# alexj94/future_urban_scene_generation

Measured on AMD Instinct MI355X. Metric: synthesised vehicle crops/sec @256x256, higher is better.
Workload: dtype f32 tensors; conv contraction as 3 fp16 MFMA products of scaled (hi, lo) operand splits, f32 accumulate (error vs fp64 <= 1.3x the exact-f32 MFMA kernel's: observed 0.96-1.27x over 12 operand scales x 5 layers; range-guarded; exact-f32 leg in precision_legs)

## Files before the change

### future_urban_scene_generation_amd/_lib.py

```python
from __future__ import annotations

import ctypes as C
import os

_HERE = os.path.dirname(os.path.abspath(__file__))
LIB_PATH = os.environ.get("FUSG_LIB", os.path.join(_HERE, "libfusg.so"))


class FusgUnavailable(RuntimeError):
    pass


class FusgError(RuntimeError):
    pass


class Tensor(C.Structure):
    _fields_ = [("data", C.c_void_p),
                ("n", C.c_int64), ("c", C.c_int64), ("h", C.c_int64), ("w", C.c_int64),
                ("sn", C.c_int64), ("sc", C.c_int64), ("sh", C.c_int64), ("sw", C.c_int64),
                ("dtype", C.c_int32), ("_pad", C.c_int32)]


class ConvDesc(C.Structure):
# ... 5 lines not shown
                ("stride", C.c_int32), ("upsample", C.c_int32), ("pad_mode", C.c_int32), ("pre_op", C.c_int32),
                ("act", C.c_int32), ("store_mode", C.c_int32), ("qh", C.c_int32), ("qw", C.c_int32),
                ("nphase", C.c_int32), ("out_sy", C.c_int32), ("out_sx", C.c_int32),
                ("out_oy", C.c_int32 * 4), ("out_ox", C.c_int32 * 4),
                ("dst_c_off", C.c_int32), ("tile", C.c_int32), ("ksplit", C.c_int32), ("precision", C.c_int32),
                ("wpack_h", C.c_void_p),
                ("kh", C.c_int32), ("kw", C.c_int32), ("dil", C.c_int32), ("pad_h", C.c_int32), ("pad_w", C.c_int32),
                ("wfrag_order", C.c_int32), ("wfrag", C.c_void_p), ("stats_out", C.c_void_p),
                ("tile_list", C.c_void_p), ("tile_count", C.c_int32), ("q_oy", C.c_int32), ("q_ox", C.c_int32),
                ("stats_slots", C.c_int32),
                ("wscale", C.c_void_p), ("status", C.c_void_p), ("wfrag_bf16", C.c_void_p), ("wfrag_f32", C.c_void_p),
                ("splitk_counters", C.c_void_p), ("splitk_counters_len", C.c_int32), ("tap_sparse", C.c_int32)]


class BneckDesc(C.Structure):
    _fields_ = [("x", Tensor), ("res", Tensor), ("dst", Tensor),
                ("pre_scale", C.c_void_p), ("pre_shift", C.c_void_p),
                ("w1frag", C.c_void_p), ("bias1", C.c_void_p), ("wscale1", C.c_void_p),
                ("w2frag", C.c_void_p), ("bias2", C.c_void_p), ("wscale2", C.c_void_p),
                ("w3frag", C.c_void_p), ("bias3", C.c_void_p), ("wscale3", C.c_void_p),
                ("status", C.c_void_p), ("planes", C.c_int32), ("exact_f32", C.c_int32)]


class RespairDesc(C.Structure):
    _fields_ = [("x", Tensor), ("s1", Tensor), ("kb", Tensor), ("kc", Tensor),
                ("w_in", C.c_void_p), ("bias_in", C.c_void_p),
                ("wfragA", C.c_void_p), ("biasA", C.c_void_p), ("wscaleA", C.c_void_p),
                ("wfragB", C.c_void_p), ("biasB", C.c_void_p), ("wscaleB", C.c_void_p),
                ("wfrag_b", C.c_void_p), ("bias_b", C.c_void_p), ("wscale_b", C.c_void_p),
                ("wfrag_c", C.c_void_p), ("bias_c", C.c_void_p), ("wscale_c", C.c_void_p),
                ("status", C.c_void_p), ("channels", C.c_int32), ("entry", C.c_int32),
                ("cin", C.c_int32), ("kpad_in", C.c_int32), ("tap_order", C.c_int32), ("_pad", C.c_int32)]


class HgHeadDesc(C.Structure):
    _fields_ = [("y_in", Tensor), ("x", Tensor), ("score", Tensor), ("dst", Tensor),
                ("wfrag_fc", C.c_void_p), ("bias_fc", C.c_void_p), ("wscale_fc", C.c_void_p),
                ("wfrag_score", C.c_void_p), ("bias_score", C.c_void_p), ("wscale_score", C.c_void_p),
                ("wfrag_join", C.c_void_p), ("bias_join", C.c_void_p), ("wscale_join", C.c_void_p),
                ("status", C.c_void_p), ("join", C.c_int32), ("_pad", C.c_int32)]


class PackSpec(C.Structure):
    _fields_ = [(n, C.c_int32) for n in ("cout", "cin", "kh", "kw", "c0", "stride", "pad", "dil", "upsample", "cin_pad")]


# ... 1 lines not shown
    _fields_ = [("cout_pad", C.c_int32), ("k_pad", C.c_int32), ("c0k", C.c_int32), ("c1k", C.c_int32),
                ("wfrag_order", C.c_int32), ("_pad", C.c_int32), ("wpack_floats", C.c_int64), ("ktab_ints", C.c_int64),
                ("wpack_h_halves", C.c_int64), ("wfrag_halves", C.c_int64)]


F32, U8, I32 = 0, 1, 2
PAD_ZERO, PAD_REFLECT, PAD_REPLICATE = 0, 1, 2
PRE_NONE, PRE_RELU, PRE_ELU, PRE_AFFINE_RELU, PRE_AFFINE = 0, 1, 2, 3, 4
ACT_NONE, ACT_RELU, ACT_TANH, ACT_SIGMOID, ACT_TANH01 = 0, 1, 2, 3, 4
STORE_NORMAL, STORE_D2S, STORE_S2D = 0, 1, 2
PREC_F32, PREC_F16X3, PREC_EMU_BF16, PREC_EMU_BF16X2, PREC_BF16 = 0, 1, 2, 3, 4
MAX_FRAMES = 64
TILE_AUTO, TILE_128x128, TILE_128x64, TILE_128x32, TILE_64x64, TILE_64x128 = 0, 1, 2, 3, 4, 5

_TP = C.POINTER(Tensor)
_SIGS = {
    "fusg_conv2d": (C.c_int, [C.POINTER(ConvDesc), C.c_void_p]),
    "fusg_conv2d_plan": (C.c_int64, [C.POINTER(ConvDesc)]),
    "fusg_conv2d_route": (C.c_int, [C.POINTER(ConvDesc)]),
    "fusg_set_route_batch": (C.c_int, [C.c_int32]),
    "fusg_route_batch": (C.c_int32, []),
    "fusg_conv2d_route_order": (C.c_int, [C.POINTER(ConvDesc), C.POINTER(C.c_int32 * 4)]),
    "fusg_hg_bottleneck": (C.c_int, [C.POINTER(BneckDesc), C.c_void_p]),
    "fusg_vunet_respair": (C.c_int, [C.POINTER(RespairDesc), C.c_void_p]),
    "fusg_hg_head": (C.c_int, [C.POINTER(HgHeadDesc), C.c_void_p]),
    "fusg_conv2d_entry_nin": (C.c_int, [C.POINTER(ConvDesc), C.POINTER(ConvDesc), C.c_void_p]),
    "fusg_conv2d_entry_nin_route": (C.c_int, [C.POINTER(ConvDesc), C.POINTER(ConvDesc)]),
    "fusg_chan_stats": (C.c_int, [_TP, C.c_void_p, C.c_int32, C.c_void_p]),
    "fusg_in_finalize": (C.c_int, [_TP, C.c_void_p, C.c_int32, C.c_float, C.c_void_p, C.c_void_p, C.c_void_p]),
    "fusg_ln_finalize": (C.c_int, [_TP, C.c_void_p, C.c_int32, C.c_float, C.c_void_p, C.c_void_p, C.c_void_p,
                                   C.c_void_p, C.c_void_p]),
    "fusg_in_finalize_slots": (C.c_int, [C.c_void_p, C.c_int32, C.c_int32, C.c_int32, C.c_float, C.c_void_p, C.c_void_p, C.c_void_p]),
    "fusg_ln_finalize_slots": (C.c_int, [C.c_void_p, C.c_int32, C.c_int32, C.c_int32, C.c_float, C.c_void_p, C.c_void_p,
                                         C.c_void_p, C.c_void_p, C.c_void_p]),
    "fusg_affine_act": (C.c_int, [_TP, C.c_void_p, C.c_void_p, C.c_int64, C.c_int32, _TP, _TP, C.c_void_p]),
    "fusg_maxpool2": (C.c_int, [_TP, _TP, C.c_void_p]),
    "fusg_upsample2_add": (C.c_int, [_TP, _TP, _TP, C.c_void_p]),
    "fusg_copy4d": (C.c_int, [_TP, _TP, C.c_int32, C.c_void_p]),
    "fusg_add4d": (C.c_int, [_TP, _TP, _TP, C.c_void_p]),
    "fusg_space_to_depth2": (C.c_int, [_TP, _TP, C.c_void_p]),
    "fusg_depth_to_space2": (C.c_int, [_TP, _TP, C.c_void_p]),
    "fusg_ec_inputs": (C.c_int, [_TP, _TP, _TP, _TP, C.c_int32, C.c_void_p]),
    "fusg_hshift_sum": (C.c_int, [_TP, C.c_void_p, C.c_int32, C.c_int32, C.c_int32, C.c_int32, _TP, C.c_void_p]),
    "fusg_argmax_hw": (C.c_int, [_TP, C.c_void_p, C.c_void_p]),
    "fusg_to_image_u8": (C.c_int, [_TP, _TP, C.c_void_p]),
    "fusg_merge_u8": (C.c_int, [_TP, _TP, _TP, _TP, C.c_void_p]),
# ... 43 lines not shown
    "fusg_plan_destroy": (None, [C.c_void_p]),
    "fusg_plan_begin": (C.c_int, [C.c_void_p]),
    "fusg_plan_end": (C.c_int, [C.c_void_p]),
    "fusg_plan_add_dependency": (C.c_int, [C.c_void_p, C.c_void_p, C.c_void_p]),
    "fusg_plan_add_h2d": (C.c_int, [C.c_void_p, C.c_void_p, C.c_void_p, C.c_int64, C.c_int32, C.c_int64, C.c_void_p]),
    "fusg_plan_next_slot": (C.c_int, [C.c_void_p]),
    "fusg_plan_size": (C.c_int64, [C.c_void_p]),
    "fusg_plan_run": (C.c_int, [C.c_void_p]),
    "fusg_plan_streams": (C.c_int32, [C.c_void_p]),
    "fusg_plan_run_mt": (C.c_int, [C.c_void_p]),
    "fusg_plan_graph_capture": (C.c_int, [C.c_void_p, C.c_void_p, C.c_int32]),
    "fusg_plan_graph_nodes": (C.c_int64, [C.c_void_p]),
    "fusg_plan_graph_slot": (C.c_int, [C.c_void_p]),
    "fusg_plan_graph_launch": (C.c_int, [C.c_void_p, C.c_void_p]),
    "fusg_pack_conv_sizes": (C.c_int, [C.POINTER(PackSpec), C.POINTER(PackSizes)]),
    "fusg_pack_conv_weights": (C.c_int, [C.POINTER(PackSpec)] + [C.c_void_p] * 8),
    "fusg_version": (C.c_int, []),
    "fusg_last_error": (C.c_char_p, []),
    "fusg_last_conv_kernel": (C.c_int, []),
    "fusg_arch": (C.c_char_p, []),
    "fusg_sizeof_tensor": (C.c_int, []),
    "fusg_sizeof_conv_desc": (C.c_int, []),
    "fusg_sizeof_bneck_desc": (C.c_int, []),
    "fusg_sizeof_respair_desc": (C.c_int, []),
    "fusg_sizeof_hg_head_desc": (C.c_int, []),
    "fusg_prof_enable": (None, [C.c_int]),
    "fusg_prof_reset": (None, []),
    "fusg_prof_read": (C.c_int, [C.c_int, C.POINTER(C.c_double), C.POINTER(C.c_int64), C.POINTER(C.c_double)]),
}
EXPORTS = tuple(_SIGS.keys())

ROUTE_BATCH_ENV = int(os.environ.get("FUSG_ROUTE_BATCH", "0") or 0)

_lib = None


def lib():
    global _lib
    if _lib is None:
        if not os.path.exists(LIB_PATH):
            raise FusgUnavailable(
                f"{LIB_PATH} not found: build it with `python -c 'import __graft_entry__ as g; g.build()'` "
                "(hipcc --offload-arch=gfx950).  There is no CPU fallback.")
        import torch
        try:
            h = C.CDLL(LIB_PATH)
        except OSError as e:
            raise FusgUnavailable(f"cannot load {LIB_PATH}: {e}") from e
        for name, (res, args) in _SIGS.items():
            fn = getattr(h, name)
            fn.restype = res
            fn.argtypes = args
        if (h.fusg_sizeof_tensor() != C.sizeof(Tensor) or h.fusg_sizeof_conv_desc() != C.sizeof(ConvDesc)
                or h.fusg_sizeof_bneck_desc() != C.sizeof(BneckDesc)
                or h.fusg_sizeof_respair_desc() != C.sizeof(RespairDesc)
                or h.fusg_sizeof_hg_head_desc() != C.sizeof(HgHeadDesc)):
            raise FusgUnavailable("libfusg.so struct layout differs from the ctypes mirror (stale build?)")
        if ROUTE_BATCH_ENV and h.fusg_set_route_batch(ROUTE_BATCH_ENV) < 0:
            raise FusgError(f"FUSG_ROUTE_BATCH={ROUTE_BATCH_ENV}: {h.fusg_last_error().decode()}")
        _lib = h
    return _lib


def check(rc: int, what: str = "") -> None:
    if rc != 0:
        msg = lib().fusg_last_error()
        raise FusgError(f"{what}: rc={rc}: {msg.decode() if msg else ''}")
```

### future_urban_scene_generation_amd/csrc/common.h

```cpp
#pragma once
#include <hip/hip_runtime.h>
#include <functional>
#include <memory>
#include <tuple>
#include <utility>
#include <stdint.h>
#include <stdio.h>
#include <string.h>
#include "../../include/fusg.h"

namespace fusg {

void set_error(const char* fmt, ...);
void note_conv_kernel(int kind);

#define FUSG_CHECK(cond, ...)                         \
    do {                                              \
        if (!(cond)) {                                \
            fusg::set_error(__VA_ARGS__);             \
            return FUSG_ERR_INVALID;                  \
        }                                             \
    } while (0)

#define FUSG_LAUNCH_CHECK(what)                                                    \
// ... 42 lines not shown

template <class A> struct SavedArg {
    A a;
    explicit SavedArg(A v) : a(v) {}
    A get() const { return a; }
};
template <> struct SavedArg<const fusg_tensor*> {
    bool has; fusg_tensor t;
    explicit SavedArg(const fusg_tensor* p) : has(p != nullptr), t(p ? *p : fusg_tensor{}) {}
    const fusg_tensor* get() const { return has ? &t : nullptr; }
};
template <> struct SavedArg<const fusg_conv_desc*> {
    bool has; fusg_conv_desc d;
    explicit SavedArg(const fusg_conv_desc* p) : has(p != nullptr), d(p ? *p : fusg_conv_desc{}) {}
    const fusg_conv_desc* get() const { return has ? &d : nullptr; }
};

template <> struct SavedArg<const fusg_bneck_desc*> {
    bool has; fusg_bneck_desc d;
    explicit SavedArg(const fusg_bneck_desc* p) : has(p != nullptr), d(p ? *p : fusg_bneck_desc{}) {}
    const fusg_bneck_desc* get() const { return has ? &d : nullptr; }
};

template <> struct SavedArg<const fusg_respair_desc*> {
    bool has; fusg_respair_desc d;
    explicit SavedArg(const fusg_respair_desc* p) : has(p != nullptr), d(p ? *p : fusg_respair_desc{}) {}
    const fusg_respair_desc* get() const { return has ? &d : nullptr; }
};

template <> struct SavedArg<const fusg_hg_head_desc*> {
    bool has; fusg_hg_head_desc d;
    explicit SavedArg(const fusg_hg_head_desc* p) : has(p != nullptr), d(p ? *p : fusg_hg_head_desc{}) {}
    const fusg_hg_head_desc* get() const { return has ? &d : nullptr; }
};

template <class... A>
int plan_dispatch(int (*impl)(A..., void*), void* stream, A... a) {
    if (plan_recording()) {
        auto saved = std::make_shared<std::tuple<SavedArg<A>...>>(SavedArg<A>(a)...);
        const int32_t rb = route_batch_now();
        plan_append((hipStream_t)stream, [impl, saved, rb](hipStream_t s) {
            RouteBatchScope scope(rb);
            return std::apply([&](const SavedArg<A>&... sv) { return impl(sv.get()..., (void*)s); }, *saved);
        });
    }
    return impl(a..., stream);
// ... 9 lines not shown
```

### future_urban_scene_generation_amd/csrc/conv_bneck.hip

```cpp
#include "conv_kernel_h3.h"

namespace fusg {

struct BneckK {
    const float* x; const float* res; float* dst;
    long xsn, xsh, xsw, rsn, rsh, rsw, dsn, dsh, dsw;
    const float* pre_scale; const float* pre_shift;
    const _Float16* w1; const _Float16* w2; const _Float16* w3;
    const float* b1; const float* b2; const float* b3;
    const float* s1; const float* s2; const float* s3;
    const float* zeros;
    int* status;
    int B, H, W, Cin, tiles_x, tiles_y;
    int touch_w;
};

constexpr int BN_HP = 100;
constexpr int BN_SROWS = 112;
constexpr size_t bneck_lds(int planes) { return (size_t)(2 * BN_SROWS * 32 + 2 * (planes / 32) * BN_HP * 32) * sizeof(_Float16); }

template <int CT> struct WFrag { h8 f[CT][2]; };

#ifdef FUSG_BNECK_STAMPS
__device__ unsigned long long g_bneck_stamps[64 * 12];
#define FUSG_STAMP(i) do { if (threadIdx.x == 0 && blockIdx.x < 64) g_bneck_stamps[blockIdx.x * 12 + (i)] = __builtin_amdgcn_s_memtime(); } while (0)
#define FUSG_STAMP_RT(i) do { if (threadIdx.x == 0 && blockIdx.x < 64) g_bneck_stamps[blockIdx.x * 12 + (i)] = __builtin_amdgcn_s_memrealtime(); } while (0)
#else
#define FUSG_STAMP(i) do {} while (0)
#define FUSG_STAMP_RT(i) do {} while (0)
#endif

__device__ __forceinline__ f32x4 mfma16(const h8 a, const h8 b, const f32x4 c) {
    return __builtin_amdgcn_mfma_f32_16x16x32_f16(a, b, c, 0, 0, 0);
}

template <int P>
__global__ __launch_bounds__(256, 2) void hg_bneck_h3(const BneckK k) {
    constexpr int NCH = P / 32;
    constexpr int CT1 = P / 64, CT3 = P / 32;
    extern __shared__ __attribute__((aligned(16))) _Float16 smem_h[];
    _Float16* Sh = smem_h;
    _Float16* Sl = Sh + BN_SROWS * 32;
    _Float16* Th = Sl + BN_SROWS * 32;
    _Float16* Tl = Th + NCH * BN_HP * 32;
    _Float16* Uh = Th;
    _Float16* Ul = Th + NCH * 64 * 32;

    const int t = threadIdx.x, lane = t & 63, wave = t >> 6;
    const int lp = lane & 15, lg = lane >> 4;
    FUSG_STAMP_RT(8);
    FUSG_STAMP(0);
    const int tile = xcd_tile();
    const int tpi = k.tiles_x * k.tiles_y;
    const int b = tile / tpi, t2 = tile - b * tpi;
    const int ty = t2 / k.tiles_x, tx = t2 - ty * k.tiles_x;
    const int oy0 = ty * 8, ox0 = tx * 8;
    float amax = 0.f;
    const float ninf = -__builtin_inff();

// ... 214 lines not shown
        for (int i = 0; i < 4; ++i) { xh[i] = *(const h8*)(Uh + c * 2048 + i * 512 + sfrag); xl[i] = *(const h8*)(Ul + c * 2048 + i * 512 + sfrag); }
        h8 bs[CT3];
#pragma unroll
        for (int j = 0; j < CT3; ++j) bs[j] = scale_m11(F.f[j][0]);
#pragma unroll
        for (int term = 0; term < 3; ++term)
#pragma unroll
            for (int i = 0; i < 4; ++i)
#pragma unroll
                for (int j = 0; j < CT3; ++j)
                    acc3[i][j] = mfma16(term == 0 ? F.f[j][0] : term == 1 ? F.f[j][1] : bs[j], term == 2 ? xl[i] : xh[i], acc3[i][j]);
    };
#pragma unroll
    for (int c = 0; c < NCH; c += 2) {
        load_w(v1, k.w3, c + 1, 2 * NCH, wave * CT3);
        compute3(v0, c);
        if (c + 2 < NCH) load_w(v0, k.w3, c + 2, 2 * NCH, wave * CT3);
        compute3(v1, c + 1);
    }

    FUSG_STAMP(6);
    if (amax >= F16X3_LIMIT && k.status) *k.status = 1;

#pragma unroll
    for (int i = 0; i < 4; ++i) {
        const int oy = oy0 + 2 * i + prow, ox = ox0 + pcol;
        if (oy >= k.H || ox >= k.W) continue;
        const float* rp = k.res + (long)b * k.rsn + (long)oy * k.rsh + (long)ox * k.rsw;
        float* dp = k.dst + (long)b * k.dsn + (long)oy * k.dsh + (long)ox * k.dsw;
#pragma unroll
        for (int j = 0; j < CT3; ++j) {
            const int n0 = (wave * CT3 + j) * 16 + lg * 4;
            const f32x4 bias = *(const f32x4*)(k.b3 + n0), wsc = *(const f32x4*)(k.s3 + n0);
            const f32x4 r = *(const f32x4*)(rp + n0);
            f32x4 v;
#pragma unroll
            for (int e = 0; e < 4; ++e) v[e] = fmaf(acc3[i][j][e], wsc[e], bias[e]) + r[e];
            *(f32x4*)(dp + n0) = v;
        }
    }
    FUSG_STAMP(7);
    FUSG_STAMP_RT(9);
}


template <int CT> struct WFragF { f32x4 f[CT][2]; };
// ... 205 lines not shown
#pragma unroll
    for (int i = 0; i < 4; ++i) {
        const int oy = oy0 + 2 * i + prow, ox = ox0 + pcol;
        if (oy >= k.H || ox >= k.W) continue;
        const float* rp = k.res + (long)b * k.rsn + (long)oy * k.rsh + (long)ox * k.rsw;
        float* dp = k.dst + (long)b * k.dsn + (long)oy * k.dsh + (long)ox * k.dsw;
#pragma unroll
        for (int j = 0; j < CT3; ++j) {
            const int n0 = (wave * CT3 + j) * 16 + lg * 4;
            const f32x4 bias = *(const f32x4*)(k.b3 + n0);
            const f32x4 r = *(const f32x4*)(rp + n0);
            f32x4 v;
#pragma unroll
            for (int e = 0; e < 4; ++e) v[e] = (acc3[i][j][e] + bias[e]) + r[e];
            *(f32x4*)(dp + n0) = v;
        }
    }
}

}

using namespace fusg;

static int bneck_impl(const fusg_bneck_desc* d, void* stream) {
    hipStream_t s = (hipStream_t)stream;
    FUSG_CHECK(d != nullptr, "hg_bottleneck: null descriptor");
    const fusg_tensor& x = d->x;
    const int P = d->planes;
    FUSG_CHECK(P == 128 || P == 64, "hg_bottleneck: planes %d (64 and 128 are built)", d->planes);
    FUSG_CHECK(is_nhwc(x) && x.c % 32 == 0 && x.c >= 32 && x.c <= 4096, "hg_bottleneck: x must be NHWC-physical f32 with c %% 32 == 0");
    FUSG_CHECK(is_nhwc(d->res) && is_nhwc(d->dst) && same_nhw(x, d->res) && same_nhw(x, d->dst) && d->res.c == 2 * P &&
               d->dst.c == 2 * P, "hg_bottleneck: res / dst must be NHWC-physical f32 [n, 2 * planes, h, w] like x");
    FUSG_CHECK(x.data != d->dst.data && d->res.data != d->dst.data, "hg_bottleneck: dst must not alias x or res (neighbouring patches read x's halo)");
    const bool f32 = d->exact_f32 == 1;
    FUSG_CHECK(d->exact_f32 == 0 || d->exact_f32 == 1, "hg_bottleneck: exact_f32 %d", d->exact_f32);
    const void* ptrs[] = {d->pre_scale, d->pre_shift, d->w1frag, d->bias1, d->w2frag, d->bias2, d->w3frag, d->bias3};
    for (const void* p : ptrs) FUSG_CHECK(p && (((uintptr_t)p) & 15) == 0, "hg_bottleneck: a parameter array is missing or not 16-byte aligned");
    if (!f32) {
        const void* sp[] = {d->wscale1, d->wscale2, d->wscale3};
        for (const void* p : sp) FUSG_CHECK(p && (((uintptr_t)p) & 15) == 0, "hg_bottleneck: a weight-scale array is missing or not 16-byte aligned");
        FUSG_CHECK(d->status != nullptr, "hg_bottleneck: status word missing");
    }
    FUSG_CHECK(x.n * x.h * x.w * x.sw < (1L << 40) && x.n >= 1 && x.h >= 1 && x.w >= 1, "hg_bottleneck: extent");
    BneckK k;
    memset(&k, 0, sizeof(k));
    k.x = (const float*)x.data; k.res = (const float*)d->res.data; k.dst = (float*)d->dst.data;
    k.xsn = x.sn; k.xsh = x.sh; k.xsw = x.sw;
    k.rsn = d->res.sn; k.rsh = d->res.sh; k.rsw = d->res.sw;
    k.dsn = d->dst.sn; k.dsh = d->dst.sh; k.dsw = d->dst.sw;
    k.pre_scale = d->pre_scale; k.pre_shift = d->pre_shift;
    k.w1 = (const _Float16*)d->w1frag; k.w2 = (const _Float16*)d->w2frag; k.w3 = (const _Float16*)d->w3frag;
    k.b1 = d->bias1; k.b2 = d->bias2; k.b3 = d->bias3;
    k.s1 = d->wscale1; k.s2 = d->wscale2; k.s3 = d->wscale3;
    k.status = d->status;
    k.zeros = zero_line();
    if (!k.zeros) { set_error("hg_bottleneck: cannot allocate the zero line"); return FUSG_ERR_LAUNCH; }
    k.B = (int)x.n; k.H = (int)x.h; k.W = (int)x.w; k.Cin = (int)x.c;
    k.tiles_x = (k.W + 7) / 8; k.tiles_y = (k.H + 7) / 8;
    const long wgs = (long)k.B * k.tiles_x * k.tiles_y;
    FUSG_CHECK(wgs < (1L << 31), "hg_bottleneck: grid");
    const void* fn = f32 ? (P == 128 ? (const void*)hg_bneck_f32<128> : (const void*)hg_bneck_f32<64>)
                         : (P == 128 ? (const void*)hg_bneck_h3<128> : (const void*)hg_bneck_h3<64>);
    const size_t lds = bneck_lds(P) + TOUCH_LDS_BYTES;
    k.touch_w = env_switches().no_touch ? 0 : 1;
    const double M = (double)x.n * x.h * x.w;
    prof_begin(0, s, 2.0 * M * ((double)x.c * P + 9.0 * P * P + 2.0 * P * P));
    const hipError_t e = launch_kernel(fn, dim3((unsigned)wgs), lds, (int)lds, k, s);
    prof_end(0, s);
    if (e != hipSuccess) { set_error("hg_bottleneck launch: %s", hipGetErrorString(e)); return FUSG_ERR_LAUNCH; }
    note_conv_kernel(FUSG_CONV_BNECK);
    return FUSG_OK;
}
extern "C" int fusg_hg_bottleneck(const fusg_bneck_desc* d, void* stream) { return fusg::plan_dispatch(bneck_impl, stream, d); }
#ifdef FUSG_BNECK_STAMPS
extern "C" int fusg_debug_bneck_stamps(unsigned long long* out) {
    return hipMemcpyFromSymbol(out, HIP_SYMBOL(fusg::g_bneck_stamps), sizeof(unsigned long long) * 64 * 12) == hipSuccess ? 0 : 1;
}
#endif
```

### future_urban_scene_generation_amd/ops.py

```python
from __future__ import annotations

import ctypes as C
from typing import Optional, Tuple

import torch

from . import _lib as L
from .pack import ConvPlan

_DT = {torch.float32: L.F32, torch.uint8: L.U8, torch.int32: L.I32}

import os as _os
import numpy as _np


def _env_set(name: str) -> bool:
    return name in _os.environ


_PREC = {"f32": L.PREC_F32, "f16x3": L.PREC_F16X3,
         "bf16": L.PREC_BF16,
         "emu_bf16": L.PREC_EMU_BF16, "emu_bf16x2": L.PREC_EMU_BF16X2}
_EMU_BITS = {"emu_bf16": 8, "emu_bf16x2": 16}

# ... 445 lines not shown
        d.stats_slots = int(buf.shape[1])
    L.check(lib.fusg_conv2d(C.byref(d), stream_ptr()), "conv2d")
    return (out, stats) if want_stats else out


def bottleneck_ok(p: dict, x: torch.Tensor, precision: Optional[str] = None) -> bool:
    prec = precision or PRECISION
    if prec not in ("f16x3", "f32") or _env_set("FUSG_NO_BNECK") or (prec == "f32" and (_env_set("FUSG_NO_BNECK_F32") or _env_set("FUSG_NO_F32_HALO"))):
        return False
    c1, c2, c3 = p["c1"], p["c2"], p["c3"]
    if not (c1.cout in (64, 128) and c2.cout == c1.cout and c3.cout == 2 * c1.cout and c1.kh == 1 and c2.kh == 3 and c3.kh == 1
            and c1.c0k == x.shape[1] and x.shape[1] % 32 == 0 and c1.c1k == 0 and c2.pad == 1 and c2.stride == 1):
        return False
    lim = _os.environ.get("FUSG_BNECK_MAXHW")
    if lim is not None and max(x.shape[2], x.shape[3]) > int(lim):
        return False
    minhw = BNECK_MINHW if BNECK_MINHW is not None else (32 if _route_n(x.shape[0]) <= 8 and prec == "f16x3" else 0)
    return max(x.shape[2], x.shape[3]) >= minhw or _env_set("FUSG_NO_SMALL")


BNECK_MINHW = int(_os.environ["FUSG_BNECK_MINHW"]) if "FUSG_BNECK_MINHW" in _os.environ else None


def bottleneck(p: dict, x: torch.Tensor, res: Optional[torch.Tensor] = None, precision: Optional[str] = None) -> torch.Tensor:
    f32 = (precision or PRECISION) == "f32"
    res = x if res is None else res
    b, _, h, w = x.shape
    planes = p["c1"].cout
    out = nhwc_empty(b, 2 * planes, h, w, x.device)
    d = L.BneckDesc()
    d.x, d.res, d.dst = desc(x), desc(res), desc(out)
    d.pre_scale, d.pre_shift = p["pre"][0].data_ptr(), p["pre"][1].data_ptr()
    if RECORDER is not None:
        RECORDER.keep.append(p["pre"])
    for i, key in ((1, "c1"), (2, "c2"), (3, "c3")):
        plan = p[key].to(x.device)
        dev = plan.dev
        if RECORDER is not None:
            RECORDER.keep.append(dev)
        assert dev.get("wfrag") is not None and dev["wfrag_order"] == 0, key
        frag = plan.frag_f32_dev() if f32 else dev["wfrag"]
        assert frag is not None, key
        if RECORDER is not None:
            RECORDER.keep.append(frag)
        setattr(d, "w%dfrag" % i, frag.data_ptr())
        setattr(d, "bias%d" % i, dev["bias"].data_ptr())
        setattr(d, "wscale%d" % i, dev["wscale"].data_ptr())
    d.status = status_word(x.device).data_ptr()
    d.planes = planes
    d.exact_f32 = 1 if f32 else 0
    L.check(L.lib().fusg_hg_bottleneck(C.byref(d), stream_ptr()), "hg_bottleneck")
    return out


VU_RESPAIR = not _env_set("FUSG_NO_RESPAIR")


def respair_ok(res_a: ConvPlan, res_b: ConvPlan, nin_b: ConvPlan, nin_c: ConvPlan, x: torch.Tensor,
               nin_in: Optional[ConvPlan] = None, precision: Optional[str] = None) -> bool:
    prec = precision or PRECISION
    if not VU_RESPAIR or prec != "f16x3" or not is_nhwc(x):
        return False
    for p in (res_a, res_b):
        if not (p.cout == 32 and p.cout_pad == 32 and p.c0k == 32 and p.c1k == 0 and p.kh == 3 and p.kw == 3 and p.pad == 1
                and p.pad_w < 0 and p.stride == 1 and p.dil == 1 and p.upsample == 0 and p.nphase == 1 and p.pad_mode == L.PAD_ZERO):
            return False
    for p in (nin_b, nin_c):
        if not (p.cout == 32 and p.cout_pad == 32 and p.c0k == 32 and p.c1k == 0 and p.kh == 1 and p.kw == 1 and p.pad == 0
                and p.stride == 1 and p.nphase == 1):
            return False
    b, c, h, w = x.shape
    if nin_in is not None:
        if not (nin_in.cout == 32 and nin_in.cout_pad == 32 and nin_in.c0k in (4, 8) and nin_in.c1k == 0 and nin_in.kh == 1
                and nin_in.kw == 1 and nin_in.pad == 0 and nin_in.stride == 1 and nin_in.nphase == 1 and c == nin_in.c_split[0]):
            return False
# ... 607 lines not shown
```

### future_urban_scene_generation_amd/stacked_hourglass/models.py

```python
from __future__ import annotations

from typing import Dict, List

import torch
import torch.nn as nn

from .. import _lib as L
from .. import ops, pack
from ..nn_base import BNP, ConvP, FusedNet, dev_vec, entry_point


class Bottleneck(nn.Module):
    expansion = 2

    def __init__(self, inplanes: int, planes: int, stride: int = 1, downsample=None):
        super().__init__()
        if stride != 1:
            raise NotImplementedError("the hourglass only instantiates stride-1 bottlenecks")
        self.bn1 = BNP(inplanes)
        self.conv1 = ConvP(inplanes, planes, 1)
        self.bn2 = BNP(planes)
        self.conv2 = ConvP(planes, planes, 3)
        self.bn3 = BNP(planes)
        self.conv3 = ConvP(planes, planes * 2, 1)
        self.downsample = downsample
# ... 80 lines not shown
             "layer3": self._pack_seq(self.layer3, device),
             "hg": [], "res": [], "fc": [], "score": [], "fc_": [], "score_": []}
        for i in range(self.num_stacks):
            P["hg"].append([[self._pack_seq(seq, device) for seq in level] for level in self.hg[i].hg])
            P["res"].append(self._pack_seq(self.res[i], device))
            wf, bf = pack.fold_bn_after_conv(self.fc[i][0].weight, self.fc[i][0].bias, *self._bn_ss(self.fc[i][1]))
            P["fc"].append(pack.pack_conv(wf, bf).to(device))
            P["score"].append(pack.pack_conv(self.score[i].weight, self.score[i].bias).to(device))
            if i < self.num_stacks - 1:
                P["fc_"].append(pack.pack_conv(self.fc_[i].weight, self.fc_[i].bias).to(device))
                P["score_"].append(pack.pack_conv(self.score_[i].weight, self.score_[i].bias).to(device))
                wj = torch.cat([self.fc_[i].weight.detach().float().cpu(), self.score_[i].weight.detach().float().cpu()], dim=1)
                bj = self.fc_[i].bias.detach().float().cpu() + self.score_[i].bias.detach().float().cpu()
                P.setdefault("join", []).append(pack.pack_conv(wj, bj, c_split=(wj.shape[1] - self.num_classes, self.num_classes),
                                                               cin_pad=32).to(device))
                ws = torch.zeros(32, self.score[i].weight.shape[1], 1, 1)
                bs = torch.zeros(32)
                ws[:self.num_classes] = self.score[i].weight.detach().float().cpu()
                bs[:self.num_classes] = self.score[i].bias.detach().float().cpu()
                P.setdefault("score32", []).append(pack.pack_conv(ws, bs).to(device))
        return P

    @staticmethod
    def _bottleneck(p: dict, x: torch.Tensor) -> torch.Tensor:
        if ops.bottleneck_ok(p, x):
            return ops.bottleneck(p, x, None if p["ds"] is None else ops.conv(p["ds"], x))
        t = ops.conv(p["c1"], x, pre_op=L.PRE_AFFINE_RELU, pre=p["pre"], act=L.ACT_RELU)
        t = ops.conv(p["c2"], t, act=L.ACT_RELU)
        r = x if p["ds"] is None else ops.conv(p["ds"], x)
        return ops.conv(p["c3"], t, res0=r)

    def _seq(self, plans: List[dict], x: torch.Tensor) -> torch.Tensor:
        for p in plans:
            x = self._bottleneck(p, x)
        return x

    def _hourglass(self, hp, n: int, x: torch.Tensor) -> torch.Tensor:
        up1 = self._seq(hp[n - 1][0], x)
        low1 = self._seq(hp[n - 1][1], ops.maxpool2(x))
        low2 = self._hourglass(hp, n - 1, low1) if n > 1 else self._seq(hp[n - 1][3], low1)
        low3 = self._seq(hp[n - 1][2], low2)
        return ops.upsample2_add(low3, up1)

    @entry_point
    def forward(self, x: torch.Tensor) -> Dict[str, List[torch.Tensor]]:
        if ops.PRECISION == "bf16":
            with ops.precision("f16x3"):
                return self._forward(x)
        return self._forward(x)

    def _forward(self, x: torch.Tensor) -> Dict[str, List[torch.Tensor]]:
        P = self._ensure(x)
        if x.dim() != 4 or x.shape[1] != 3 or x.shape[2] % 64 or x.shape[3] % 64:
            raise ValueError(f"HourglassNet expects [B,3,H,W] with H,W multiples of 64, got {tuple(x.shape)}")
        heatmaps = []
        x = ops.conv(P["stem"], ops.as_nhwc(x), act=L.ACT_RELU)
        x = self._seq(P["layer1"], x)
        x = ops.maxpool2(x)
        x = self._seq(P["layer2"], x)
        x = self._seq(P["layer3"], x)
        for i in range(self.num_stacks):
            y = self._hourglass(P["hg"][i], 4, x)
            y = self._seq(P["res"][i], y)
            last = i == self.num_stacks - 1
            sp, jp = (P["score"][i], None) if last else (P["score32"][i], P["join"][i])
            if ops.hg_head_ok(P["fc"][i], sp, y, jp, x):
                score, xn = ops.hg_head(P["fc"][i], sp, y, jp, x)
                heatmaps.append(ops.to_nchw(score[:, :self.num_classes]))
                x = x if last else xn
                continue
            y = ops.conv(P["fc"][i], y, act=L.ACT_RELU)
            joined = not last and ops.halo_precision() and y.shape[1] % 32 == 0 and self.num_classes <= 32
            score = ops.conv(P["score32"][i], y)[:, :self.num_classes] if joined else ops.conv(P["score"][i], y)
            heatmaps.append(ops.to_nchw(score))
            if joined:
                x = ops.conv(P["join"][i], y, score, res0=x)
            elif not last:
                t = ops.conv(P["fc_"][i], y, res0=x)
                x = ops.conv(P["score_"][i], score, res0=t)
        return {"heatmaps": heatmaps}


def get_maxima_device(heatmaps: torch.Tensor):
    import numpy as np
    b, c, h, w = heatmaps.shape
# ... 6 lines not shown
```

### include/fusg.h

```cpp
#ifndef FUSG_H
#define FUSG_H

#include <stdint.h>

#ifdef __cplusplus
extern "C" {
#endif

#define FUSG_VERSION 118

typedef enum fusg_status {
    FUSG_OK = 0,
    FUSG_ERR_INVALID = -1,
    FUSG_ERR_LAUNCH = -2,
    FUSG_ERR_UNSUPPORTED = -3
} fusg_status;

typedef enum fusg_dtype { FUSG_F32 = 0, FUSG_U8 = 1, FUSG_I32 = 2 } fusg_dtype;

typedef struct fusg_tensor {
    void*   data;
    int64_t n, c, h, w;
    int64_t sn, sc, sh, sw;
    int32_t dtype;
// ... 81 lines not shown
} fusg_conv_desc;

int  fusg_conv2d(const fusg_conv_desc* d, void* stream);
int64_t fusg_conv2d_plan(fusg_conv_desc* d);
int  fusg_conv2d_route(const fusg_conv_desc* d);

int     fusg_set_route_batch(int32_t n);
int32_t fusg_route_batch(void);
int  fusg_conv2d_route_order(const fusg_conv_desc* d, int32_t out[4]);

typedef struct fusg_bneck_desc {
    fusg_tensor x, res, dst;
    const float* pre_scale;
    const float* pre_shift;
    const void*  w1frag; const float* bias1; const float* wscale1;
    const void*  w2frag; const float* bias2; const float* wscale2;
    const void*  w3frag; const float* bias3; const float* wscale3;
    int32_t*     status;
    int32_t      planes;
    int32_t      exact_f32;
} fusg_bneck_desc;
int fusg_hg_bottleneck(const fusg_bneck_desc* d, void* stream);

typedef struct fusg_respair_desc {
    fusg_tensor x, s1, kb, kc;
    const float* w_in; const float* bias_in;
    const void*  wfragA;  const float* biasA;  const float* wscaleA;
    const void*  wfragB;  const float* biasB;  const float* wscaleB;
    const void*  wfrag_b; const float* bias_b; const float* wscale_b;
    const void*  wfrag_c; const float* bias_c; const float* wscale_c;
    int32_t*     status;
    int32_t      channels;
    int32_t      entry;
    int32_t      cin, kpad_in;
    int32_t      tap_order;
    int32_t      _pad;
} fusg_respair_desc;
int fusg_vunet_respair(const fusg_respair_desc* d, void* stream);

int fusg_conv2d_entry_nin(const fusg_conv_desc* res, const fusg_conv_desc* nin, void* stream);
int fusg_conv2d_entry_nin_route(const fusg_conv_desc* res, const fusg_conv_desc* nin);

typedef struct fusg_hg_head_desc {
    fusg_tensor y_in, x, score, dst;
    const void*  wfrag_fc;    const float* bias_fc;    const float* wscale_fc;
    const void*  wfrag_score; const float* bias_score; const float* wscale_score;
// ... 187 lines not shown
int        fusg_plan_graph_capture(fusg_plan* p, void* capture_stream, int32_t slot);
int64_t    fusg_plan_graph_nodes(const fusg_plan* p);
int        fusg_plan_graph_slot(fusg_plan* p);
int        fusg_plan_graph_launch(fusg_plan* p, void* stream);


int         fusg_version(void);
const char* fusg_last_error(void);
enum { FUSG_CONV_GENERIC_F32 = 0, FUSG_CONV_GENERIC_F16X3 = 1, FUSG_CONV_HALO = 2, FUSG_CONV_HALO_S2D = 3,
       FUSG_CONV_TAPUNIT = 4, FUSG_CONV_HALO_BF16 = 5, FUSG_CONV_BNECK = 6 ,
       FUSG_CONV_POINTWISE = 7 ,
       FUSG_CONV_SMALL = 8 ,
       FUSG_CONV_HALO_F32 = 9 ,
       FUSG_CONV_TAPUNIT_F32 = 10 ,
       FUSG_CONV_TAPUNIT_BF16 = 11 ,
       FUSG_CONV_RESPAIR = 12 ,
       FUSG_CONV_HALO_ENTRY = 13 ,
       FUSG_CONV_HG_HEAD = 14  };
int         fusg_last_conv_kernel(void);
const char* fusg_arch(void);
int         fusg_sizeof_tensor(void);
int         fusg_sizeof_conv_desc(void);
int         fusg_sizeof_bneck_desc(void);
int         fusg_sizeof_respair_desc(void);
int         fusg_sizeof_hg_head_desc(void);
void fusg_prof_enable(int on);
void fusg_prof_reset(void);
int  fusg_prof_read(int kind, double* total_ms, int64_t* launches, double* flops);

#ifdef __cplusplus
}
#endif
#endif
```

Measured before the change: 1518.

## Fuse downsample projection and 2x2 maxpool into the hourglass bottleneck kernel

Adds a GLUE variant of the split-fp16 bottleneck kernel. It computes the 1x1 downsample projection in-kernel from an LDS-staged hi/lo split of the input, replacing the separate ds conv launch and its residual tensor round trip. It can also emit the 2x2 max-pooled output directly using DPP lane shuffles, so separate maxpool launches are dropped and, for layer1, the full-resolution output write is skipped. The costs are more LDS pressure and register use in the fused kernel, an extra route probe for eligibility, and a larger kernel to maintain.

```diff
diff --git a/future_urban_scene_generation_amd/_lib.py b/future_urban_scene_generation_amd/_lib.py
--- a/future_urban_scene_generation_amd/_lib.py
+++ b/future_urban_scene_generation_amd/_lib.py
@@ -51,6 +51,11 @@
                 ("status", C.c_void_p), ("planes", C.c_int32), ("exact_f32", C.c_int32)]
 
 
+class BneckExDesc(C.Structure):
+    _fields_ = [("b", BneckDesc), ("pool_dst", Tensor),
+                ("wds_frag", C.c_void_p), ("bias_ds", C.c_void_p), ("wscale_ds", C.c_void_p)]
+
+
 class RespairDesc(C.Structure):
     _fields_ = [("x", Tensor), ("s1", Tensor), ("kb", Tensor), ("kc", Tensor),
                 ("w_in", C.c_void_p), ("bias_in", C.c_void_p),
@@ -98,6 +103,7 @@
     "fusg_route_batch": (C.c_int32, []),
     "fusg_conv2d_route_order": (C.c_int, [C.POINTER(ConvDesc), C.POINTER(C.c_int32 * 4)]),
     "fusg_hg_bottleneck": (C.c_int, [C.POINTER(BneckDesc), C.c_void_p]),
+    "fusg_hg_bottleneck_ex": (C.c_int, [C.POINTER(BneckExDesc), C.c_void_p]),
     "fusg_vunet_respair": (C.c_int, [C.POINTER(RespairDesc), C.c_void_p]),
     "fusg_hg_head": (C.c_int, [C.POINTER(HgHeadDesc), C.c_void_p]),
     "fusg_conv2d_entry_nin": (C.c_int, [C.POINTER(ConvDesc), C.POINTER(ConvDesc), C.c_void_p]),
@@ -187,6 +193,7 @@
     "fusg_sizeof_tensor": (C.c_int, []),
     "fusg_sizeof_conv_desc": (C.c_int, []),
     "fusg_sizeof_bneck_desc": (C.c_int, []),
+    "fusg_sizeof_bneck_ex_desc": (C.c_int, []),
     "fusg_sizeof_respair_desc": (C.c_int, []),
     "fusg_sizeof_hg_head_desc": (C.c_int, []),
     "fusg_prof_enable": (None, [C.c_int]),
@@ -218,6 +225,7 @@
             fn.argtypes = args
         if (h.fusg_sizeof_tensor() != C.sizeof(Tensor) or h.fusg_sizeof_conv_desc() != C.sizeof(ConvDesc)
                 or h.fusg_sizeof_bneck_desc() != C.sizeof(BneckDesc)
+                or h.fusg_sizeof_bneck_ex_desc() != C.sizeof(BneckExDesc)
                 or h.fusg_sizeof_respair_desc() != C.sizeof(RespairDesc)
                 or h.fusg_sizeof_hg_head_desc() != C.sizeof(HgHeadDesc)):
             raise FusgUnavailable("libfusg.so struct layout differs from the ctypes mirror (stale build?)")
diff --git a/future_urban_scene_generation_amd/csrc/common.h b/future_urban_scene_generation_amd/csrc/common.h
--- a/future_urban_scene_generation_amd/csrc/common.h
+++ b/future_urban_scene_generation_amd/csrc/common.h
@@ -88,6 +88,12 @@
     const fusg_bneck_desc* get() const { return has ? &d : nullptr; }
 };
 
+template <> struct SavedArg<const fusg_bneck_ex_desc*> {
+    bool has; fusg_bneck_ex_desc d;
+    explicit SavedArg(const fusg_bneck_ex_desc* p) : has(p != nullptr), d(p ? *p : fusg_bneck_ex_desc{}) {}
+    const fusg_bneck_ex_desc* get() const { return has ? &d : nullptr; }
+};
+
 template <> struct SavedArg<const fusg_respair_desc*> {
     bool has; fusg_respair_desc d;
     explicit SavedArg(const fusg_respair_desc* p) : has(p != nullptr), d(p ? *p : fusg_respair_desc{}) {}
diff --git a/future_urban_scene_generation_amd/csrc/conv_bneck.hip b/future_urban_scene_generation_amd/csrc/conv_bneck.hip
--- a/future_urban_scene_generation_amd/csrc/conv_bneck.hip
+++ b/future_urban_scene_generation_amd/csrc/conv_bneck.hip
@@ -13,6 +13,10 @@
     int* status;
     int B, H, W, Cin, tiles_x, tiles_y;
     int touch_w;
+    const _Float16* wds; const float* bds; const float* sds;
+    float* pool;
+    long psn, psh, psw;
+    float vfloor;
 };
 
 constexpr int BN_HP = 100;
@@ -34,7 +38,14 @@
     return __builtin_amdgcn_mfma_f32_16x16x32_f16(a, b, c, 0, 0, 0);
 }
 
-template <int P>
+__device__ __forceinline__ float dpp_xor1(float v) {
+    return __builtin_bit_cast(float, __builtin_amdgcn_update_dpp(0, __builtin_bit_cast(int, v), 0xB1, 0xF, 0xF, true));
+}
+__device__ __forceinline__ float dpp_xor8(float v) {
+    return __builtin_bit_cast(float, __builtin_amdgcn_update_dpp(0, __builtin_bit_cast(int, v), 0x128, 0xF, 0xF, true));
+}
+
+template <int P, bool GLUE = false>
 __global__ __launch_bounds__(256, 2) void hg_bneck_h3(const BneckK k) {
     constexpr int NCH = P / 32;
     constexpr int CT1 = P / 64, CT3 = P / 32;
@@ -295,6 +306,124 @@
     FUSG_STAMP(6);
     if (amax >= F16X3_LIMIT && k.status) *k.status = 1;
 
+    if constexpr (GLUE) {
+        const bool ds = k.wds != nullptr;
+        _Float16* Xh = smem_h;
+        _Float16* Xl = Xh + nch1 * 2048;
+        if (ds) {
+            __syncthreads();
+            load_w(v0, k.wds, 0, 2 * NCH, wave * CT3);
+            {
+                const float* xq[2];
+                int xo[2];
+                bool okx[2];
+#pragma unroll
+                for (int j = 0; j < 2; ++j) {
+                    const int p = (t >> 3) + 32 * j;
+                    const int oy = oy0 + (p >> 3), ox = ox0 + (p & 7);
+                    okx[j] = oy < k.H && ox < k.W;
+                    xq[j] = okx[j] ? k.x + (long)b * k.xsn + (long)oy * k.xsh + (long)ox * k.xsw + kc * 4 : k.zeros;
+                    xo[j] = p * 32 + ((((kc >> 1) ^ (((p >> 2) & 1) << 1)) << 3) | ((kc & 1) << 2));
+                }
+                for (int c0 = 0; c0 < nch1; c0 += 4) {
+                    f32x4 r[4][2];
+#pragma unroll
+                    for (int u = 0; u < 4; ++u)
+#pragma unroll
+                        for (int j = 0; j < 2; ++j) r[u][j] = *(const f32x4*)((okx[j] && c0 + u < nch1) ? xq[j] + (c0 + u) * 32 : k.zeros);
+#pragma unroll
+                    for (int u = 0; u < 4; ++u)
+                        if (c0 + u < nch1) {
+#pragma unroll
+                            for (int j = 0; j < 2; ++j) {
+                                h4 hi, lo;
+                                split4(r[u][j], k.vfloor, hi, lo, amax);
+                                *(h4*)(Xh + (c0 + u) * 2048 + xo[j]) = hi;
+                                *(h4*)(Xl + (c0 + u) * 2048 + xo[j]) = lo;
+                            }
+                        }
+                }
+            }
+            if (amax >= F16X3_LIMIT && k.status) *k.status = 1;
+            __syncthreads();
+        }
+
+        const bool full = k.dst != nullptr, pool = k.pool != nullptr;
+#pragma unroll
+        for (int hp = 0; hp < 2; ++hp) {
+            f32x4 accd[2][CT3];
+#pragma unroll
+            for (int i = 0; i < 2; ++i)
+#pragma unroll
+                for (int j = 0; j < CT3; ++j) accd[i][j] = f32x4{0.f, 0.f, 0.f, 0.f};
+            if (ds) {
+                auto computed = [&](const WFrag<CT3>& F, int c) {
+                    h8 xh[2], xl[2];
+#pragma unroll
+                    for (int i = 0; i < 2; ++i) {
+                        xh[i] = *(const h8*)(Xh + c * 2048 + (2 * hp + i) * 512 + sfrag);
+                        xl[i] = *(const h8*)(Xl + c * 2048 + (2 * hp + i) * 512 + sfrag);
+                    }
+                    h8 bs[CT3];
+#pragma unroll
+                    for (int j = 0; j < CT3; ++j) bs[j] = scale_m11(F.f[j][0]);
+#pragma unroll
+                    for (int term = 0; term < 3; ++term)
+#pragma unroll
+                        for (int i = 0; i < 2; ++i)
+#pragma unroll
+                            for (int j = 0; j < CT3; ++j)
+                                accd[i][j] = mfma16(term == 0 ? F.f[j][0] : term == 1 ? F.f[j][1] : bs[j], term == 2 ? xl[i] : xh[i], accd[i][j]);
+                };
+                for (int c = 0; c < nch1; c += 2) {
+                    if (c + 1 < nch1) load_w(v1, k.wds, c + 1, 2 * NCH, wave * CT3);
+                    computed(v0, c);
+                    if (c + 1 >= nch1) break;
+                    if (c + 2 < nch1) load_w(v0, k.wds, c + 2, 2 * NCH, wave * CT3);
+                    computed(v1, c + 1);
+                }
+                if (hp == 0) load_w(v0, k.wds, 0, 2 * NCH, wave * CT3);
+            }
+#pragma unroll
+            for (int ii = 0; ii < 2; ++ii) {
+                const int i = 2 * hp + ii;
+                const int oy = oy0 + 2 * i + prow, ox = ox0 + pcol;
+                const bool in = oy < k.H && ox < k.W;
+                const bool pst = in && (lp & 9) == 0;
+                const float* rp = (in && !ds) ? k.res + (long)b * k.rsn + (long)oy * k.rsh + (long)ox * k.rsw : k.zeros;
+                float* dp = k.dst + (long)b * k.dsn + (long)oy * k.dsh + (long)ox * k.dsw;
+                float* pp = k.pool + (long)b * k.psn + (long)(oy >> 1) * k.psh + (long)(ox >> 1) * k.psw;
+#pragma unroll
+                for (int j = 0; j < CT3; ++j) {
+                    const int n0 = (wave * CT3 + j) * 16 + lg * 4;
+                    const f32x4 bias = *(const f32x4*)(k.b3 + n0), wsc = *(const f32x4*)(k.s3 + n0);
+                    f32x4 r;
+                    if (ds) {
+                        const f32x4 bd = *(const f32x4*)(k.bds + n0), sd = *(const f32x4*)(k.sds + n0);
+#pragma unroll
+                        for (int e = 0; e < 4; ++e) r[e] = fmaf(accd[ii][j][e], sd[e], bd[e]);
+                    } else {
+                        r = *(const f32x4*)(in ? rp + n0 : rp);
+                    }
+                    f32x4 v;
+#pragma unroll
+                    for (int e = 0; e < 4; ++e) v[e] = fmaf(acc3[i][j][e], wsc[e], bias[e]) + r[e];
+                    if (full && in) *(f32x4*)(dp + n0) = v;
+                    if (pool) {
+                        f32x4 m;
+#pragma unroll
+                        for (int e = 0; e < 4; ++e) {
+                            const float ab = fmaxf(v[e], dpp_xor1(v[e]));
+                            m[e] = fmaxf(ab, dpp_xor8(ab));
+                        }
+                        if (pst) *(f32x4*)(pp + n0) = m;
+                    }
+                }
+            }
+        }
+        return;
+    }
+
 #pragma unroll
     for (int i = 0; i < 4; ++i) {
         const int oy = oy0 + 2 * i + prow, ox = ox0 + pcol;
@@ -546,18 +675,40 @@
 
 using namespace fusg;
 
-static int bneck_impl(const fusg_bneck_desc* d, void* stream) {
+static int bneck_launch(const fusg_bneck_desc* d, const fusg_bneck_ex_desc* ex, void* stream) {
     hipStream_t s = (hipStream_t)stream;
     FUSG_CHECK(d != nullptr, "hg_bottleneck: null descriptor");
     const fusg_tensor& x = d->x;
     const int P = d->planes;
+    const bool ds = ex && ex->wds_frag != nullptr, pool = ex && ex->pool_dst.data != nullptr;
+    const bool glue = ds || pool, full = !pool || d->dst.data != nullptr;
     FUSG_CHECK(P == 128 || P == 64, "hg_bottleneck: planes %d (64 and 128 are built)", d->planes);
     FUSG_CHECK(is_nhwc(x) && x.c % 32 == 0 && x.c >= 32 && x.c <= 4096, "hg_bottleneck: x must be NHWC-physical f32 with c %% 32 == 0");
-    FUSG_CHECK(is_nhwc(d->res) && is_nhwc(d->dst) && same_nhw(x, d->res) && same_nhw(x, d->dst) && d->res.c == 2 * P &&
-               d->dst.c == 2 * P, "hg_bottleneck: res / dst must be NHWC-physical f32 [n, 2 * planes, h, w] like x");
-    FUSG_CHECK(x.data != d->dst.data && d->res.data != d->dst.data, "hg_bottleneck: dst must not alias x or res (neighbouring patches read x's halo)");
+    FUSG_CHECK(d->exact_f32 == 0 || d->exact_f32 == 1, "hg_bottleneck: exact_f32 %d", d->exact_f32);
+    if (glue && d->exact_f32 == 1) {
+        set_error("hg_bottleneck_ex: the ds projection and the pooled store are built for split-fp16 only (exact_f32 = 1 keeps the separate launches)");
+        return FUSG_ERR_UNSUPPORTED;
+    }
+    if (!ds) FUSG_CHECK(is_nhwc(d->res) && same_nhw(x, d->res) && d->res.c == 2 * P,
+                        "hg_bottleneck: res must be NHWC-physical f32 [n, 2 * planes, h, w] like x");
+    if (full) {
+        FUSG_CHECK(is_nhwc(d->dst) && same_nhw(x, d->dst) && d->dst.c == 2 * P, "hg_bottleneck: dst must be NHWC-physical f32 [n, 2 * planes, h, w] like x");
+        FUSG_CHECK(x.data != d->dst.data && (ds || d->res.data != d->dst.data), "hg_bottleneck: dst must not alias x or res (neighbouring patches read x's halo)");
+    }
+    if (ds) {
+        const void* pd[] = {ex->wds_frag, ex->bias_ds, ex->wscale_ds};
+        for (const void* p : pd) FUSG_CHECK(p && (((uintptr_t)p) & 15) == 0, "hg_bottleneck_ex: a ds parameter array is missing or not 16-byte aligned");
+        FUSG_CHECK((size_t)(x.c / 32) * 64 * 32 * 2 * sizeof(_Float16) <= bneck_lds(P),
+                   "hg_bottleneck_ex: the split patch of %ld input channels does not fit the block's LDS", (long)x.c);
+    }
+    if (pool) {
+        const fusg_tensor& q = ex->pool_dst;
+        FUSG_CHECK(x.h % 2 == 0 && x.w % 2 == 0, "hg_bottleneck_ex: the pooled store needs even h and w");
+        FUSG_CHECK(is_nhwc(q) && q.n == x.n && q.c == 2 * P && 2 * q.h == x.h && 2 * q.w == x.w,
+                   "hg_bottleneck_ex: pool_dst must be NHWC-physical f32 [n, 2 * planes, h / 2, w / 2]");
+        FUSG_CHECK(q.data != x.data && q.data != d->dst.data && (ds || q.data != d->res.data), "hg_bottleneck_ex: pool_dst aliases x, res or dst");
+    }
     const bool f32 = d->exact_f32 == 1;
-    FUSG_CHECK(d->exact_f32 == 0 || d->exact_f32 == 1, "hg_bottleneck: exact_f32 %d", d->exact_f32);
     const void* ptrs[] = {d->pre_scale, d->pre_shift, d->w1frag, d->bias1, d->w2frag, d->bias2, d->w3frag, d->bias3};
     for (const void* p : ptrs) FUSG_CHECK(p && (((uintptr_t)p) & 15) == 0, "hg_bottleneck: a parameter array is missing or not 16-byte aligned");
     if (!f32) {
@@ -583,19 +734,33 @@
     k.tiles_x = (k.W + 7) / 8; k.tiles_y = (k.H + 7) / 8;
     const long wgs = (long)k.B * k.tiles_x * k.tiles_y;
     FUSG_CHECK(wgs < (1L << 31), "hg_bottleneck: grid");
+    if (glue) {
+        k.vfloor = -__builtin_inff();
+        if (!full) { k.dst = nullptr; k.dsn = k.dsh = k.dsw = 0; }
+        if (ds) { k.res = nullptr; k.wds = (const _Float16*)ex->wds_frag; k.bds = ex->bias_ds; k.sds = ex->wscale_ds; }
+        if (pool) { k.pool = (float*)ex->pool_dst.data; k.psn = ex->pool_dst.sn; k.psh = ex->pool_dst.sh; k.psw = ex->pool_dst.sw; }
+    }
     const void* fn = f32 ? (P == 128 ? (const void*)hg_bneck_f32<128> : (const void*)hg_bneck_f32<64>)
-                         : (P == 128 ? (const void*)hg_bneck_h3<128> : (const void*)hg_bneck_h3<64>);
+                   : glue ? (P == 128 ? (const void*)hg_bneck_h3<128, true> : (const void*)hg_bneck_h3<64, true>)
+                          : (P == 128 ? (const void*)hg_bneck_h3<128> : (const void*)hg_bneck_h3<64>);
     const size_t lds = bneck_lds(P) + TOUCH_LDS_BYTES;
     k.touch_w = env_switches().no_touch ? 0 : 1;
     const double M = (double)x.n * x.h * x.w;
-    prof_begin(0, s, 2.0 * M * ((double)x.c * P + 9.0 * P * P + 2.0 * P * P));
+    prof_begin(0, s, 2.0 * M * ((double)x.c * P + 9.0 * P * P + 2.0 * P * P + (ds ? 2.0 * x.c * P : 0.0)));
     const hipError_t e = launch_kernel(fn, dim3((unsigned)wgs), lds, (int)lds, k, s);
     prof_end(0, s);
     if (e != hipSuccess) { set_error("hg_bottleneck launch: %s", hipGetErrorString(e)); return FUSG_ERR_LAUNCH; }
     note_conv_kernel(FUSG_CONV_BNECK);
     return FUSG_OK;
 }
+static int bneck_impl(const fusg_bneck_desc* d, void* stream) { return bneck_launch(d, nullptr, stream); }
+static int bneck_ex_impl(const fusg_bneck_ex_desc* d, void* stream) {
+    FUSG_CHECK(d != nullptr, "hg_bottleneck_ex: null descriptor");
+    return bneck_launch(&d->b, d, stream);
+}
 extern "C" int fusg_hg_bottleneck(const fusg_bneck_desc* d, void* stream) { return fusg::plan_dispatch(bneck_impl, stream, d); }
+extern "C" int fusg_hg_bottleneck_ex(const fusg_bneck_ex_desc* d, void* stream) { return fusg::plan_dispatch(bneck_ex_impl, stream, d); }
+extern "C" int fusg_sizeof_bneck_ex_desc(void) { return (int)sizeof(fusg_bneck_ex_desc); }
 #ifdef FUSG_BNECK_STAMPS
 extern "C" int fusg_debug_bneck_stamps(unsigned long long* out) {
     return hipMemcpyFromSymbol(out, HIP_SYMBOL(fusg::g_bneck_stamps), sizeof(unsigned long long) * 64 * 12) == hipSuccess ? 0 : 1;
diff --git a/future_urban_scene_generation_amd/ops.py b/future_urban_scene_generation_amd/ops.py
--- a/future_urban_scene_generation_amd/ops.py
+++ b/future_urban_scene_generation_amd/ops.py
@@ -491,14 +491,48 @@
 BNECK_MINHW = int(_os.environ["FUSG_BNECK_MINHW"]) if "FUSG_BNECK_MINHW" in _os.environ else None
 
 
-def bottleneck(p: dict, x: torch.Tensor, res: Optional[torch.Tensor] = None, precision: Optional[str] = None) -> torch.Tensor:
+BNECK_GLUE = not _env_set("FUSG_NO_BNECK_GLUE")
+
+
+def bottleneck_glue_ok(p: dict, x: torch.Tensor, ds: Optional[ConvPlan] = None, pool: bool = False,
+                       precision: Optional[str] = None) -> bool:
+    prec = precision or PRECISION
+    if not BNECK_GLUE or prec != "f16x3" or not is_nhwc(x) or not bottleneck_ok(p, x, prec):
+        return False
+    b, c, h, w = x.shape
+    if pool and (h % 2 or w % 2):
+        return False
+    if ds is None:
+        return True
+    planes = p["c1"].cout
+    if not (_k1(ds, c, 0) and ds.cout == 2 * planes and ds.cout_pad == ds.cout and (c // 32) * 8192 <= (39936 if planes == 64 else 65536)):
+        return False
+    key = (b, c, h, w, x.stride(3), str(x.device), ROUTE_BATCH,
+           _env_set("FUSG_NO_SMALL"), _env_set("FUSG_NO_POINTWISE"), _env_set("FUSG_SMALL_KSPLIT"))
+    memo = ds.__dict__.setdefault("_bneck_glue_routes", {})
+    if key not in memo:
+        t = nhwc_empty(1, ds.cout, 8, 16, x.device)
+        d, _ = _conv_desc(ds, x, out=t, precision=prec)
+        tt = d.dst
+        tt.n, tt.h, tt.w, tt.sh, tt.sn = b, h, w, w * tt.sw, h * w * tt.sw
+        L.lib().fusg_conv2d_plan(C.byref(d))
+        order = (C.c_int32 * 4)()
+        rc = L.lib().fusg_conv2d_route_order(C.byref(d), C.byref(order))
+        memo[key] = rc == 0 and order[0] == 2 and order[2] <= 1 and order[3] == 0
+    return memo[key]
+
+
+def bottleneck(p: dict, x: torch.Tensor, res: Optional[torch.Tensor] = None, precision: Optional[str] = None, *,
+               ds: Optional[ConvPlan] = None, pool: bool = False, keep_full: bool = True):
     f32 = (precision or PRECISION) == "f32"
     res = x if res is None else res
     b, _, h, w = x.shape
     planes = p["c1"].cout
-    out = nhwc_empty(b, 2 * planes, h, w, x.device)
-    d = L.BneckDesc()
-    d.x, d.res, d.dst = desc(x), desc(res), desc(out)
+    glue = ds is not None or pool
+    out = nhwc_empty(b, 2 * planes, h, w, x.device) if keep_full or not pool else None
+    dx = L.BneckExDesc() if glue else None
+    d = dx.b if glue else L.BneckDesc()
+    d.x, d.res, d.dst = desc(x), desc(None if ds is not None else res), desc(out)
     d.pre_scale, d.pre_shift = p["pre"][0].data_ptr(), p["pre"][1].data_ptr()
     if RECORDER is not None:
         RECORDER.keep.append(p["pre"])
@@ -518,8 +552,21 @@
     d.status = status_word(x.device).data_ptr()
     d.planes = planes
     d.exact_f32 = 1 if f32 else 0
-    L.check(L.lib().fusg_hg_bottleneck(C.byref(d), stream_ptr()), "hg_bottleneck")
-    return out
+    if not glue:
+        L.check(L.lib().fusg_hg_bottleneck(C.byref(d), stream_ptr()), "hg_bottleneck")
+        return out
+    pooled = None
+    if ds is not None:
+        dev = ds.to(x.device).dev
+        if RECORDER is not None:
+            RECORDER.keep.append(dev)
+        assert dev.get("wfrag") is not None and dev["wfrag_order"] == 0, "ds"
+        dx.wds_frag, dx.bias_ds, dx.wscale_ds = dev["wfrag"].data_ptr(), dev["bias"].data_ptr(), dev["wscale"].data_ptr()
+    if pool:
+        pooled = nhwc_empty(b, 2 * planes, h // 2, w // 2, x.device)
+        dx.pool_dst = desc(pooled)
+    L.check(L.lib().fusg_hg_bottleneck_ex(C.byref(dx), stream_ptr()), "hg_bottleneck_ex")
+    return out if not pool else ((out, pooled) if keep_full else pooled)
 
 
 VU_RESPAIR = not _env_set("FUSG_NO_RESPAIR")
diff --git a/future_urban_scene_generation_amd/stacked_hourglass/models.py b/future_urban_scene_generation_amd/stacked_hourglass/models.py
--- a/future_urban_scene_generation_amd/stacked_hourglass/models.py
+++ b/future_urban_scene_generation_amd/stacked_hourglass/models.py
@@ -1,6 +1,6 @@
 from __future__ import annotations
 
-from typing import Dict, List
+from typing import Dict, List, Optional
 
 import torch
 import torch.nn as nn
@@ -127,23 +127,37 @@
         return P
 
     @staticmethod
-    def _bottleneck(p: dict, x: torch.Tensor) -> torch.Tensor:
+    def _bottleneck(p: dict, x: torch.Tensor, pool: bool = False, keep_full: bool = True):
         if ops.bottleneck_ok(p, x):
-            return ops.bottleneck(p, x, None if p["ds"] is None else ops.conv(p["ds"], x))
+            ds = p["ds"]
+            fuse_ds = ds is not None and ops.bottleneck_glue_ok(p, x, ds=ds)
+            fuse_pool = pool and ops.bottleneck_glue_ok(p, x, pool=True)
+            res = None if ds is None or fuse_ds else ops.conv(ds, x)
+            r = ops.bottleneck(p, x, res, ds=ds if fuse_ds else None, pool=fuse_pool, keep_full=keep_full)
+            if not pool:
+                return r
+            return (r, None) if not fuse_pool else (r if keep_full else (None, r))
         t = ops.conv(p["c1"], x, pre_op=L.PRE_AFFINE_RELU, pre=p["pre"], act=L.ACT_RELU)
         t = ops.conv(p["c2"], t, act=L.ACT_RELU)
         r = x if p["ds"] is None else ops.conv(p["ds"], x)
-        return ops.conv(p["c3"], t, res0=r)
-
-    def _seq(self, plans: List[dict], x: torch.Tensor) -> torch.Tensor:
-        for p in plans:
+        out = ops.conv(p["c3"], t, res0=r)
+        return (out, None) if pool else out
+
+    def _seq(self, plans: List[dict], x: torch.Tensor, pool: bool = False, keep_full: bool = True):
+        for p in plans[:-1]:
             x = self._bottleneck(p, x)
-        return x
-
-    def _hourglass(self, hp, n: int, x: torch.Tensor) -> torch.Tensor:
+        return self._bottleneck(plans[-1], x, pool, keep_full)
+
+    def _hourglass(self, hp, n: int, x: torch.Tensor, xp: Optional[torch.Tensor] = None) -> torch.Tensor:
         up1 = self._seq(hp[n - 1][0], x)
-        low1 = self._seq(hp[n - 1][1], ops.maxpool2(x))
-        low2 = self._hourglass(hp, n - 1, low1) if n > 1 else self._seq(hp[n - 1][3], low1)
+        if xp is None:
+            xp = ops.maxpool2(x)
+        if n > 1:
+            low1, low1p = self._seq(hp[n - 1][1], xp, pool=True)
+            low2 = self._hourglass(hp, n - 1, low1, low1p)
+        else:
+            low1 = self._seq(hp[n - 1][1], xp)
+            low2 = self._seq(hp[n - 1][3], low1)
         low3 = self._seq(hp[n - 1][2], low2)
         return ops.upsample2_add(low3, up1)
 
@@ -160,12 +174,13 @@
             raise ValueError(f"HourglassNet expects [B,3,H,W] with H,W multiples of 64, got {tuple(x.shape)}")
         heatmaps = []
         x = ops.conv(P["stem"], ops.as_nhwc(x), act=L.ACT_RELU)
-        x = self._seq(P["layer1"], x)
-        x = ops.maxpool2(x)
+        full, x = self._seq(P["layer1"], x, pool=True, keep_full=False)
+        if x is None:
+            x = ops.maxpool2(full)
         x = self._seq(P["layer2"], x)
-        x = self._seq(P["layer3"], x)
+        x, xp = self._seq(P["layer3"], x, pool=True)
         for i in range(self.num_stacks):
-            y = self._hourglass(P["hg"][i], 4, x)
+            y = self._hourglass(P["hg"][i], 4, x, xp if i == 0 else None)
             y = self._seq(P["res"][i], y)
             last = i == self.num_stacks - 1
             sp, jp = (P["score"][i], None) if last else (P["score32"][i], P["join"][i])
diff --git a/include/fusg.h b/include/fusg.h
--- a/include/fusg.h
+++ b/include/fusg.h
@@ -127,6 +127,13 @@
 } fusg_bneck_desc;
 int fusg_hg_bottleneck(const fusg_bneck_desc* d, void* stream);
 
+typedef struct fusg_bneck_ex_desc {
+    fusg_bneck_desc b;
+    fusg_tensor  pool_dst;
+    const void*  wds_frag; const float* bias_ds; const float* wscale_ds;
+} fusg_bneck_ex_desc;
+int fusg_hg_bottleneck_ex(const fusg_bneck_ex_desc* d, void* stream);
+
 typedef struct fusg_respair_desc {
     fusg_tensor x, s1, kb, kc;
     const float* w_in; const float* bias_in;
@@ -360,6 +367,7 @@
 int         fusg_sizeof_tensor(void);
 int         fusg_sizeof_conv_desc(void);
 int         fusg_sizeof_bneck_desc(void);
+int         fusg_sizeof_bneck_ex_desc(void);
 int         fusg_sizeof_respair_desc(void);
 int         fusg_sizeof_hg_head_desc(void);
 void fusg_prof_enable(int on);
```

New measurement: 1531, median of 6. About the same (+0.9%).
